# qdrant/qdrant

Hardware: AMD Instinct MI355X
Metric: QPS @ recall@10, brute-force, d=768 10M vecs, f32 cosine top-10 (higher is better)
Workload: dtype f32 (int8 prefilter + exact f32 re-score)

## Files before the change

### qdrant_amd/csrc/api_core.hip

```cpp
#include "api_internal.hpp"

namespace qmx {

static thread_local std::string g_last_error;
const std::string &last_error_text() { return g_last_error; }

void set_error(const char *fmt, ...) {
    char buf[1024];
    va_list ap;
    va_start(ap, fmt);
    vsnprintf(buf, sizeof(buf), fmt, ap);
    va_end(ap);
    g_last_error = buf;
}

int32_t hip_status(hipError_t e, const char *what, const char *file, int line) {
    set_error("HIP error %d (%s) at %s:%d: %s", (int)e, hipGetErrorString(e), file, line, what);
    (void)hipGetLastError();
    switch (e) {
        case hipErrorOutOfMemory: return QMX_ERR_OUT_OF_MEMORY;
        case hipErrorNoDevice:
        case hipErrorInvalidDevice:
        case hipErrorNoBinaryForGpu:
        case hipErrorInsufficientDriver: return QMX_ERR_NO_DEVICE;
        case hipErrorNotReady: return QMX_ERR_NOT_READY;
        case hipErrorInvalidValue: return QMX_ERR_BAD_ARG;
        default: return QMX_ERR_OTHER;
    }
}

static const char *const g_option_names[OPT_COUNT] = {"no_mfma_scan", "no_mfma16", "no_prescan", "prescan_shift", "hnsw_log_cap", "no_split_scan", "split_min_queries", "no_split256", "no_pq_pair", "no_pq_prefilter", "pq_prefilter_min_queries", "hnsw_pq_per_cu", "tq_rotate_block", "no_topk_small", "verify_max_per_query", "hnsw_pq_direct_walk", "hnsw_pq_table_build", "hnsw_no_pq_prefilter", "hnsw_no_lds_visited", "pq_lut_no_lds", "hnsw_per_cu", "hnsw_reference_heap_order", "tq_wide_min_queries", "tq_wide_high_digit", "sq_wide_min_queries", "i8_resident", "debug"};
struct OptionTable {
    std::atomic<int64_t> v[OPT_COUNT];
    int64_t initial[OPT_COUNT];
    OptionTable() {
        for (int i = 0; i < OPT_COUNT; ++i) {
            char env[64] = "QMX_";
            size_t k = 4;
            for (const char *c = g_option_names[i]; *c && k + 1 < sizeof(env); ++c) env[k++] = (char)toupper((unsigned char)*c);
            env[k] = 0;
            const char *e = getenv(env);
            int64_t val = 0;
            if (e) { val = (*e >= '0' && *e <= '9') ? atoll(e) : 1; }
            if (i == OPT_PRESCAN_SHIFT && !e) val = 10;
            if (i == OPT_SPLIT_MIN_QUERIES && !e) val = 1;
            if (i == OPT_PQ_PREFILTER_MIN_QUERIES && !e) val = 4;
            if (i == OPT_TQ_WIDE_MIN_QUERIES && !e) val = 33;
            if (i == OPT_SQ_WIDE_MIN_QUERIES && !e) val = 33;
            if (i == OPT_I8_RESIDENT && !e) val = 1;
            initial[i] = val;
            v[i].store(val, std::memory_order_relaxed);
        }
    }
};
static OptionTable g_options;
int64_t option(Option o) { return g_options.v[o].load(std::memory_order_relaxed); }

static thread_local const void *g_last_kernel = nullptr;
const void *last_noted_kernel() { return g_last_kernel; }
void note_kernel(const void *host_function) { g_last_kernel = host_function; }

void clear_stale_error() {
    hipError_t e = hipGetLastError();
    if (e != hipSuccess) {
        const bool debug = option(OPT_DEBUG) != 0;
        if (debug) fprintf(stderr, "[qmx] dropped stale HIP error %d (%s) before a kernel launch\n", (int)e, hipGetErrorString(e));
    }
}

bool is_device_ptr(const void *p) {
    if (!p) return false;
    hipPointerAttribute_t attr;
// ... 90 lines not shown
```

### qdrant_amd/csrc/api_internal.hpp

```cpp
#pragma once
#include <stdarg.h>
#include <stdio.h>
#include <stdlib.h>
#include <string.h>

#include <ctype.h>
#include <cxxabi.h>

#include <algorithm>
#include <atomic>
#include <mutex>
#include <string>
#include <thread>
#include <new>
#include <vector>

#include "kernels.hpp"
#include "tq_rotate.hpp"

namespace qmx {
const std::string &last_error_text();
const void *last_noted_kernel();
bool is_device_ptr(const void *p);
uint32_t elem_bytes(uint32_t dtype);
// ... 345 lines not shown
    DeletedView del;
};

struct CustomWalk {
    const qmx_custom_query *d_desc;
    const float *d_coefs;
    uint32_t n_queries, max_examples;
    uint32_t lds_bytes = 0;
};

static bool tq_l1(const qmx_segment *s) { return s->dtype == QMX_DTYPE_TQ && s->distance == QMX_DISTANCE_MANHATTAN; }

extern "C" {
int32_t hnsw_enqueue(const qmx_hnsw *g, qmx_query *q, uint32_t top, uint32_t ef, qmx_scored_point *d_out,
                            uint32_t *d_counts, uint32_t *d_scored, bool timed, bool acorn = false, const MultiWalk *mw = nullptr,
                            const ExpandedOut *xo = nullptr, const CustomWalk *cw = nullptr, const PopTrace *pt = nullptr);
int32_t hnsw_check(const qmx_hnsw *g, const qmx_query *q, uint32_t top, uint32_t ef);
int32_t hnsw_search_sync(const qmx_hnsw *g, qmx_query *q, uint32_t top, uint32_t ef, qmx_scored_point *out, uint32_t *out_counts,
                                const volatile uint8_t *is_stopped, qmx_counters *counters, bool acorn);
void fill_args(const qmx_query *q, uint32_t tile0, uint32_t nq_tile, ScanArgs &a);
int32_t launch_scan(const qmx_query *q, int qt, ScanMode mode, const ScanArgs &a, uint32_t *grid);
int32_t tq_l1_scores_device(qmx_query *q, uint32_t q0, uint32_t nq, const uint32_t *d_ids, uint64_t n, float *d_scores, uint64_t stride, const PairSel *sel);
int32_t score_matrix_enqueue(const qmx_query *q, uint32_t tile0, uint32_t nq_tile, const uint32_t *d_ids, uint64_t n, float *d_scores, uint64_t stride,
                                    uint32_t *launches);
int32_t score_ids_device(qmx_query *q, const uint32_t *d_ids, uint64_t n, float *d_scores, qmx_counters *counters);
int32_t score_pairs_device(qmx_query *q, const PairSel &sel, const uint32_t *d_ids, uint64_t n_items, float *d_scores,
                                  bool timed);
int32_t search_enqueue(qmx_query *q, uint32_t top, const uint32_t *d_ids, uint64_t n_ids,
                              qmx_scored_point *d_out, uint32_t *d_counts, const volatile uint8_t *is_stopped,
                              qmx_counters *counters, bool timed);
int32_t fold_split_counters(qmx_query *q, qmx_counters *c);
int32_t custom_validate(const qmx_query *ex, const qmx_custom_query *queries, uint32_t n_queries, uint32_t n_examples, uint32_t *max_examples);
TqRotationHost tq_rotation(const qmx_segment *s);
TqRotationHost tq_rotation_inverse(const qmx_segment *s);
}
void sparse_segment_free(qmx_segment *s);
void sparse_query_free(qmx_query *q);
int32_t sparse_query_create_internal(const qmx_segment *seg, const uint32_t *point_ids, uint32_t nq, qmx_query **out);
int32_t sparse_score_matrix(const qmx_query *q, uint32_t tile0, uint32_t nq_tile, const uint32_t *d_ids, uint64_t n, float *d_scores, uint64_t stride);
int32_t sparse_score_pairs(qmx_query *q, const PairSel &sel, const uint32_t *d_ids, uint64_t n_items, float *d_scores);
int32_t sparse_score_internal(const qmx_segment *seg, const uint32_t *a_ids, const uint32_t *b_ids, uint32_t n, float *out);
int32_t sparse_search_enqueue(qmx_query *q, uint32_t top, const uint32_t *d_ids, uint64_t n_ids, qmx_scored_point *d_out, uint32_t *d_counts,
                              const volatile uint8_t *is_stopped, qmx_counters *counters, bool timed);
```

### qdrant_amd/csrc/api_query.hip

```cpp
#include "api_internal.hpp"

extern "C" {

static int32_t query_alloc(const qmx_segment *seg, uint32_t nq, qmx_query **out, bool internal = false) {
    qmx_query *q = new (std::nothrow) qmx_query();
    QMX_REQUIRE(q, QMX_ERR_OUT_OF_MEMORY, "host allocation failed");
    q->seg = seg;
    q->device = seg->device;
    q->nq = nq;
    q->nq_padded = ((nq + MAX_QT_TOPK - 1) / MAX_QT_TOPK) * MAX_QT_TOPK;
    if (q->nq_padded == 0) q->nq_padded = MAX_QT_TOPK;
    if (seg->dtype == QMX_DTYPE_PQ) q->nq_padded = std::max<uint32_t>(nq, 1);
    q->bq_bits = (seg->dtype == QMX_DTYPE_BQ && !internal) ? seg->bq_query_bits : 1;
    q->aux_off = (uint32_t)((seg->scan_dim * elem_bytes(seg->dtype) * q->bq_bits + 127) & ~127u);
    if (seg->dtype == QMX_DTYPE_TQ) tq_entry_layout(seg, &q->bq_bits, &q->tq_qbytes_off, &q->aux_off);
    if (seg->dtype == QMX_DTYPE_BQ && q->bq_bits > 1 && seg->fast_layout()) {
        q->tq_qbytes_off = q->aux_off;
        q->aux_off += ((seg->scan_dim + 63) & ~63u) * 8;
    }
    q->q_stride = q->aux_off + QUERY_AUX_BYTES;
    if (seg->dtype == QMX_DTYPE_SQ_U8 || seg->dtype == QMX_DTYPE_F16 || seg->dtype == QMX_DTYPE_TQ || (seg->dtype == QMX_DTYPE_BQ && q->tq_qbytes_off))
        q->q_stride = lds_tile_stride(q->q_stride);
    if (seg->dtype == QMX_DTYPE_PQ) {
        q->q_stride = (uint32_t)(((size_t)seg->pq_m * seg->pq.n_centroids * sizeof(float) + 15) & ~(size_t)15);
// ... 335 lines not shown
    }
    set_error("dtype %u not built yet", s->dtype);
    return QMX_ERR_NOT_SUPPORTED;
}

int32_t tq_l1_scores_device(qmx_query *q, uint32_t q0, uint32_t nq, const uint32_t *d_ids, uint64_t n, float *d_scores, uint64_t stride, const PairSel *sel) {
    const qmx_segment *s = q->seg;
    const uint64_t B = 65536;
    QMX_TRY(q->tq_rot.reserve((size_t)std::min<uint64_t>(n, B) * s->tq_padded_dim * sizeof(double)));
    double *buf = (double *)q->tq_rot.p;
    const float *d_q = (const float *)q->enc.p + (size_t)q0 * s->dim;
    for (uint64_t r0 = 0; r0 < n; r0 += B) {
        const uint32_t cnt = (uint32_t)std::min<uint64_t>(B, n - r0);
        QMX_TRY(launch_tq_l1_dequant(q->stream, s->d_rows, s->row_stride, s->d_tq_sf, d_ids ? d_ids + r0 : nullptr, r0, cnt, s->n, s->tq_padded_dim, s->tq_value_bits,
                                     s->d_tq_shift, s->d_tq_scale, buf, q->d_err, sel));
        QMX_TRY(launch_tq_rotate_f64(q->stream, buf, cnt, tq_rotation_inverse(s)));
        QMX_TRY(launch_tq_l1_scores(q->stream, buf, cnt, s->tq_padded_dim, s->dim, sel ? (const float *)q->enc.p : d_q, s->dim, 0, nq, d_scores, stride, r0,
                                    s->tq_invert ? 1 : 0, sel, r0));
    }
    return QMX_OK;
}

int32_t score_matrix_enqueue(const qmx_query *q, uint32_t tile0, uint32_t nq_tile, const uint32_t *d_ids, uint64_t n, float *d_scores, uint64_t stride,
                                    uint32_t *launches) {
    const qmx_segment *s = q->seg;
    if (is_sparse(s)) {
        if (launches) ++*launches;
        return sparse_score_matrix(q, tile0, nq_tile, d_ids, n, d_scores, stride);
    }
    if (tq_l1(s)) {
        if (launches) *launches += 3 * (uint32_t)((n + 65535) / 65536);
        return tq_l1_scores_device(const_cast<qmx_query *>(q), tile0, nq_tile, d_ids, n, d_scores, stride, nullptr);
    }
    const uint32_t SQT = tile_qt(s, q);
    const bool loops = s->dtype == QMX_DTYPE_F32 && SQT >= 8 && mfma_scan_ok(s);
    const uint32_t step = loops ? nq_tile : SQT;
    for (uint32_t st0 = 0; st0 < nq_tile; st0 += step) {
        const uint32_t nq_sub = std::min<uint32_t>(step, nq_tile - st0);
        ScanArgs pre;
        fill_args(q, tile0 + st0, nq_sub, pre);
        pre.ids = d_ids;
        pre.n_cand = n;
        pre.top = 1;
        pre.scores = d_scores + (size_t)st0 * stride;
        pre.scores_stride = stride;
        uint32_t pgrid = 0;
        QMX_TRY(launch_scan(q, (int)std::min<uint32_t>(pow2_ceil(nq_sub), std::max<uint32_t>(SQT, 8)), SCAN_SCORES, pre, &pgrid));
        if (launches) ++*launches;
    }
    return QMX_OK;
}

int32_t score_ids_device(qmx_query *q, const uint32_t *d_ids, uint64_t n, float *d_scores, qmx_counters *counters) {
    const qmx_segment *s = q->seg;
    const uint32_t TQ = tile_qt(s, q);
    uint32_t launches = 0;
    QMX_TRY(score_matrix_enqueue(q, 0, q->nq, d_ids, n, d_scores, n, &launches));
    if (counters) {
        counters->kernel_launches += launches;
        counters->vectors_scored += (uint64_t)q->nq * n;
        counters->bytes_read += (uint64_t)((q->nq + TQ - 1) / TQ) * n * s->row_bytes;
    }
    return QMX_OK;
}

int32_t qmx_score_points(qmx_query *q, const uint32_t *ids, uint32_t n, float *scores, qmx_counters *counters) {
    QMX_REQUIRE(q && (n == 0 || (ids && scores)), QMX_ERR_BAD_ARG, "NULL argument");
    QMX_HIP(hipSetDevice(q->seg->device));
    if (counters) memset(counters, 0, sizeof(*counters));
    if (n == 0 || q->nq == 0) return QMX_OK;
// ... 269 lines not shown
```

### qdrant_amd/csrc/api_search.hip

```cpp
#include "api_internal.hpp"

extern "C" {



static int32_t split_stage(qmx_query *q, const char *what) {
    if (option(OPT_DEBUG) < 2) return QMX_OK;
    hipError_t e = hipStreamSynchronize(q->stream);
    fprintf(stderr, "[qmx] split stage %-28s %s\n", what, e == hipSuccess ? "ok" : hipGetErrorString(e));
    fflush(stderr);
    return e == hipSuccess ? QMX_OK : QMX_ERR_OTHER;
}

static int32_t verify_pool(qmx_query *q, unsigned char *plan, VerifyPool *vp) {
    const uint32_t cap = (uint32_t)std::min<uint64_t>(std::max<uint64_t>((uint64_t)q->nq * SPLIT_VCAP, 262144), 1u << 26);
    QMX_TRY(q->sp_ver.reserve(((size_t)cap * 2 + (size_t)q->nq * 2) * 4));
    QMX_TRY(q->sp_vscores.reserve((size_t)cap * 4));
    uint32_t *b = (uint32_t *)q->sp_ver.p;
    vp->ids = b;
    vp->qsel = b + cap;
    vp->off = b + (size_t)2 * cap;
    vp->cnt = vp->off + q->nq;
    vp->used = (uint32_t *)(plan + 24);
    vp->cap = cap;
// ... 344 lines not shown
            ::qmx::clear_stale_error();
            hipLaunchKernelGGL(sample_ids_kernel, dim3((uint32_t)((S + 255) / 256)), dim3(256), 0, q->stream, (uint32_t *)q->sp_sample.p, (uint32_t)S, n_cand / S);
            QMX_HIP(hipGetLastError());
            q->sp_sample_n = S;
            q->sp_sample_of = n_cand;
        }
        QMX_HIP(hipMemsetAsync(plan, 0, pl.zero_bytes, q->stream));
    }
    for (uint32_t tile0 = 0; tile0 < q->nq; tile0 += TQ) {
        const uint32_t nq_tile = std::min<uint32_t>(TQ, q->nq - tile0);
        if (split && (nq_tile > MAX_QT_TOPK || s->d_rows_split)) {
            if (is_stopped && *is_stopped) {
                set_error("search cancelled");
                return QMX_ERR_CANCELLED;
            }
            const uint32_t S = (uint32_t)q->sp_sample_n;
            const uint32_t *d_sample = (const uint32_t *)q->sp_sample.p;
            uint64_t *gthr = (uint64_t *)q->gthr.p + tile0;
            ScanArgs a;
            fill_args(q, tile0, nq_tile, a);
            a.n_cand = n_cand;
            a.top = top;
            QMX_TRY(q->scores.reserve((size_t)nq_tile * S * sizeof(float)));
            QMX_TRY(score_matrix_enqueue(q, tile0, nq_tile, d_sample, S, (float *)q->scores.p, S, nullptr));
            QMX_TRY(launch_custom_topk(q->stream, (const float *)q->scores.p, S, d_sample, a.del, nq_tile, top, d_out + (size_t)tile0 * top, d_counts + tile0, gthr));
            QMX_TRY(split_stage(q, "prescan"));
            if (s->split_i8) {
                float *sp_texact = sp_qnorm, *sp_qscale = sp_qmax;
                QMX_TRY(launch_split_i8_pack(q->stream, (const float *)q->enc.p + (size_t)tile0 * s->dim, nq_tile, s->dim, s->d_i8_scale, gthr, s->d_i8_stats,
                                             s->row_norm_max, q->sp_bq.p, sp_qscale, sp_band, sp_thr, sp_texact, (uint32_t *)q->sp_cnt.p, SPLIT_QT_MAX));
                QMX_TRY(split_stage(q, "int8 pack"));
                const uint32_t np = split_i8_probe();
                uint32_t *probe_ids = (uint32_t *)q->sp_probe.p, *probe_cnt = probe_ids + (size_t)q->nq * np;
                int *tile_ovf = (int *)(plan + pl.tile_ovf) + split_tiles.size();
                const uint32_t sstride = 16;
                for (uint32_t ph = 1; ph <= 2; ++ph) {
                    const uint32_t phase = ph | (sstride << 8);
                    size_t slot = 0;
                    if (timed) QMX_TRY(timing_begin(q, &slot));
                    QMX_TRY(launch_scan_i8copy(q->stream, a, q->sp_bq.p, sp_qscale, sp_thr, s->num_cus, s->d_rows_split, q->sp_wl.p, phase));
                    q->last_kernel = last_noted_kernel();
                    if (timed) QMX_TRY(timing_end(q, slot));
                    QMX_TRY(launch_split_regroup(q->stream, a, q->sp_wl.p, s->num_cus, (uint64_t *)q->sp_cand.p, (uint32_t *)q->sp_cnt.p, SPLIT_CAND_CAP, tile_ovf,
                                                 phase, SPLIT_QT));
                    QMX_TRY(launch_split_i8_probe(q->stream, (const uint64_t *)q->sp_cand.p, (const uint32_t *)q->sp_cnt.p, SPLIT_CAND_CAP, sp_band, nq_tile, top, tile_ovf,
                                                  probe_ids + (size_t)tile0 * np, probe_cnt + tile0));
                    const void *scan_kernel = q->last_kernel;
                    PairSel psel{nullptr, np, probe_cnt};
// ... 373 lines not shown
```

### qdrant_amd/csrc/common.hpp

```cpp
#pragma once
#include <hip/hip_runtime.h>
#include <hip/hip_fp16.h>
#include <stdint.h>
#include <atomic>
#include <string>

#include "../../include/qdrant_amd.h"

namespace qmx {

void set_error(const char *fmt, ...);
int32_t hip_status(hipError_t e, const char *what, const char *file, int line);
void clear_stale_error();

enum Option {
    OPT_NO_MFMA_SCAN = 0,
    OPT_NO_MFMA16,
    OPT_NO_PRESCAN,
    OPT_PRESCAN_SHIFT,
    OPT_HNSW_LOG_CAP,
    OPT_NO_SPLIT_SCAN,
    OPT_SPLIT_MIN_QUERIES,
    OPT_NO_SPLIT256,
    OPT_NO_PQ_PAIR,
    OPT_NO_PQ_PREFILTER,
    OPT_PQ_PREFILTER_MIN_QUERIES,
    OPT_HNSW_PQ_PER_CU,
    OPT_TQ_ROTATE_BLOCK,
    OPT_NO_TOPK_SMALL,
    OPT_VERIFY_MAX_PER_QUERY,
    OPT_HNSW_PQ_DIRECT_WALK,
    OPT_HNSW_PQ_TABLE_BUILD,
    OPT_HNSW_NO_PQ_PREFILTER,
    OPT_HNSW_NO_LDS_VISITED,
    OPT_PQ_LUT_NO_LDS,
    OPT_HNSW_PER_CU,
    OPT_HNSW_REFERENCE_HEAP_ORDER,
    OPT_TQ_WIDE_MIN_QUERIES,
    OPT_TQ_WIDE_HIGH_DIGIT,
    OPT_SQ_WIDE_MIN_QUERIES,
    OPT_I8_RESIDENT,
    OPT_DEBUG,
    OPT_COUNT
};
int64_t option(Option o);
struct DeviceOnce {
    std::atomic<uint64_t> done{0};
    int dev = 0;
    bool need() {
        if (hipGetDevice(&dev) != hipSuccess) { dev = 0; return true; }
        return dev >= 64 || !(done.load(std::memory_order_acquire) & (1ull << dev));
    }
    void mark() { if (dev < 64) done.fetch_or(1ull << dev, std::memory_order_release); }
};
void note_kernel(const void *host_function);
#define QMX_NOTE_KERNEL(fn) ::qmx::note_kernel(reinterpret_cast<const void *>(fn))

#define QMX_HIP(expr)                                                        \
    do {                                                                     \
        hipError_t e__ = (expr);                                             \
        if (e__ != hipSuccess) return ::qmx::hip_status(e__, #expr, __FILE__, __LINE__); \
    } while (0)

#define QMX_TRY(expr)                           \
// ... 99 lines not shown
```

### qdrant_amd/csrc/custom_query.hip

```cpp
#include "custom_combine.hpp"
#include "kernels.hpp"

namespace qmx {

__device__ __forceinline__ float custom_combine(const qmx_custom_query &q, const float *sims, uint64_t stride, const float *coefs) {
    const float *s = sims + (uint64_t)q.first * stride;
    return custom_score_by(q.kind, q.n_a, q.n_b, coefs + q.coef_first, [&](uint32_t e) { return s[(uint64_t)e * stride]; });
}

__global__ __launch_bounds__(256) void custom_combine_kernel(const qmx_custom_query *queries, uint32_t n_queries, const float *sims, uint64_t n,
                                                             const float *coefs, float *out) {
    const uint64_t c = (uint64_t)blockIdx.x * 256 + threadIdx.x;
    const uint32_t qi = blockIdx.y;
    if (c >= n || qi >= n_queries) return;
    out[(uint64_t)qi * n + c] = custom_combine(queries[qi], sims + c, n, coefs);
}

int32_t launch_custom_combine(hipStream_t st, const qmx_custom_query *d_queries, uint32_t n_queries, const float *d_sims, uint64_t n,
                              const float *d_coefs, float *d_out) {
    if (n == 0 || n_queries == 0) return QMX_OK;
    ::qmx::clear_stale_error();
    hipLaunchKernelGGL(custom_combine_kernel, dim3((uint32_t)((n + 255) / 256), n_queries), dim3(256), 0, st, d_queries, n_queries, d_sims, n, d_coefs, d_out);
    QMX_HIP(hipGetLastError());
    return QMX_OK;
// ... 124 lines not shown
            }
            const uint32_t cnt = (uint32_t)__popcll(__ballot(ok));
            if (lane == 0) {
                sh_bound = cnt == (uint32_t)ptop ? readlane_u64(merged, ptop - 1) : 0ull;
                total += cnt;
            }
            total = (uint32_t)__builtin_amdgcn_readfirstlane((int)total);
        }
        __syncthreads();
        bound = sh_bound;
        if (bound == 0) {
            for (uint32_t i = off + WAVE + threadIdx.x; i < top; i += CT_BLOCK) out[(uint64_t)q * top + i] = qmx_scored_point{0u, 0.0f};
            break;
        }
    }
    if (threadIdx.x == 0) {
        out_counts[q] = total;
        if (bound_out) bound_out[q] = total == top ? bound : 0ull;
    }
}

constexpr int CTS_E = 16;
constexpr uint64_t CTS_MAX_N = (uint64_t)CT_BLOCK * CTS_E;
__global__ __launch_bounds__(CT_BLOCK) void custom_topk_small_kernel(const float *scores, uint32_t n, const uint32_t *ids, DeletedView del, uint32_t top,
                                                                     qmx_scored_point *out, uint32_t *out_counts, uint64_t *bound_out) {
    extern __shared__ __attribute__((aligned(16))) unsigned char smem_cts[];
    uint64_t *surv = reinterpret_cast<uint64_t *>(smem_cts);
    __shared__ uint64_t sh_t[CT_NW];
    __shared__ uint64_t sh_bound;
    __shared__ uint32_t sh_cnt;
    const uint32_t q = blockIdx.x;
    const int lane = threadIdx.x & 63, wave = threadIdx.x >> 6;
    const float *row = scores + (uint64_t)q * n;
    uint64_t kreg[CTS_E];
#pragma unroll
    for (int e0 = 0; e0 < CTS_E; e0 += 8) {
        if ((uint32_t)e0 * CT_BLOCK >= n) {
#pragma unroll
            for (int u = 0; u < 8; ++u) kreg[e0 + u] = 0ull;
            continue;
        }
        uint32_t id[8];
        uint64_t key[8], keep[8];
#pragma unroll
        for (int u = 0; u < 8; ++u) {
            const uint32_t c = (uint32_t)(e0 + u) * CT_BLOCK + threadIdx.x;
            const uint32_t cc = c < n ? c : 0;
            id[u] = ids ? ids[cc] : cc;
            key[u] = c < n ? make_key(row[cc], id[u]) : 0ull;
        }
        live_masks<8>(del, id, keep);
#pragma unroll
        for (int u = 0; u < 8; ++u) kreg[e0 + u] = key[u] & keep[u];
    }
    uint64_t bound = ~0ull;
    uint32_t total = 0;
    for (uint32_t off = 0; off < top; off += WAVE) {
        const uint32_t ptop = top - off < (uint32_t)WAVE ? top - off : (uint32_t)WAVE;
        uint64_t m = 0;
#pragma unroll
        for (int e = 0; e < CTS_E; ++e) {
            const uint64_t k = kreg[e] < bound ? kreg[e] : 0ull;
            m = k > m ? k : m;
        }
        uint32_t rank = 0;
        for (int j = 0; j < WAVE; ++j) rank += readlane_u64(m, j) > m ? 1u : 0u;
        const uint64_t sel = __ballot(rank == ptop - 1 && m != 0);
        const uint64_t tw = sel ? readlane_u64(m, __builtin_ctzll(sel)) : 0ull;
        if (lane == 0) sh_t[wave] = tw;
        if (threadIdx.x == 0) { sh_cnt = 0; sh_bound = 0; }
        __syncthreads();
        uint64_t t = 0;
#pragma unroll
        for (int w = 0; w < CT_NW; ++w) t = sh_t[w] > t ? sh_t[w] : t;
#pragma unroll
        for (int e = 0; e < CTS_E; ++e) {
            const uint64_t k = kreg[e] < bound ? kreg[e] : 0ull;
            if (k != 0 && k >= t) surv[atomicAdd(&sh_cnt, 1u)] = k;
        }
        __syncthreads();
        const uint32_t cnt = sh_cnt;
        for (uint32_t i = threadIdx.x; i < cnt; i += CT_BLOCK) {
            const uint64_t my = surv[i];
            uint32_t r = 0;
            for (uint32_t j = 0; j < cnt; ++j) r += (surv[j] > my || (surv[j] == my && j < i)) ? 1u : 0u;
            if (r < ptop) {
                qmx_scored_point p;
                p.idx = key_idx(my);
                p.score = key_score(my);
                out[(uint64_t)q * top + off + r] = p;
                if (r == ptop - 1) sh_bound = my;
            }
        }
        const uint32_t found = cnt < ptop ? cnt : ptop;
        for (uint32_t i = found + threadIdx.x; i < ptop; i += CT_BLOCK) out[(uint64_t)q * top + off + i] = qmx_scored_point{0u, 0.0f};
        total += found;
        __syncthreads();
        bound = sh_bound;
        if (bound == 0) {
            for (uint32_t i = off + WAVE + threadIdx.x; i < top; i += CT_BLOCK) out[(uint64_t)q * top + i] = qmx_scored_point{0u, 0.0f};
            break;
        }
        __syncthreads();
    }
    if (threadIdx.x == 0) {
        out_counts[q] = total;
        if (bound_out) bound_out[q] = total == top ? bound : 0ull;
    }
}

int32_t launch_custom_topk(hipStream_t st, const float *d_scores, uint64_t n, const uint32_t *d_ids, const DeletedView &del, uint32_t n_queries,
                           uint32_t top, qmx_scored_point *d_out, uint32_t *d_counts, uint64_t *d_bound) {
    if (n_queries == 0) return QMX_OK;
    ::qmx::clear_stale_error();
    if (n >= 1 && n <= CTS_MAX_N && !option(OPT_NO_TOPK_SMALL)) {
        static thread_local DeviceOnce attr_once;
        if (attr_once.need()) {
            QMX_HIP(hipFuncSetAttribute(reinterpret_cast<const void *>(custom_topk_small_kernel), hipFuncAttributeMaxDynamicSharedMemorySize, (int)(CTS_MAX_N * 8)));
            attr_once.mark();
        }
        hipLaunchKernelGGL(custom_topk_small_kernel, dim3(n_queries), dim3(CT_BLOCK), (size_t)n * 8, st, d_scores, (uint32_t)n, d_ids, del, top, d_out, d_counts, d_bound);
        QMX_HIP(hipGetLastError());
        return QMX_OK;
    }
    hipLaunchKernelGGL(custom_topk_kernel, dim3(n_queries), dim3(CT_BLOCK), 0, st, d_scores, n, d_ids, del, top, d_out, d_counts, d_bound);
    QMX_HIP(hipGetLastError());
    return QMX_OK;
}

}
```

### qdrant_amd/csrc/kernels.hpp

```cpp
#pragma once
#include "common.hpp"

namespace qmx {

constexpr int MAX_QT = 16;
constexpr int SCAN_BLOCK = 512;
constexpr int MAX_TOP_FAST = 64;

struct TqEc {
    const int16_t *weights;
    const float *xm;
    float weight_scale, mm_const;
};
struct ScanArgs {
    const void *rows;
    uint64_t n_rows;
    uint64_t row_stride;
    uint32_t dim;
    uint32_t nseg;
    uint32_t rem_pieces;
    uint32_t tail_start;
    uint32_t aux_off;
    uint32_t nq;
    const void *queries;
// ... 196 lines not shown
    uint32_t *next;
};
int32_t launch_hnsw_build_bq(hipStream_t st, const ScanArgs &a, const HnswBuildArgs &h, int phase, uint32_t grid, int *per_cu);
int32_t launch_hnsw_build_sq(hipStream_t st, int distance, const ScanArgs &a, const HnswBuildArgs &h, int phase, uint32_t grid, int *per_cu);
int32_t launch_hnsw_build_dense(hipStream_t st, int dtype, int distance, const ScanArgs &a, const HnswBuildArgs &h, int phase,
                                uint32_t grid, int *per_cu);
int32_t launch_hnsw_build_maxsim_dense(hipStream_t st, int dtype, int distance, const ScanArgs &a, const HnswBuildArgs &h, int phase, uint32_t grid,
                                       int *per_cu);
int32_t launch_hnsw_build_maxsim_sq(hipStream_t st, int distance, const ScanArgs &a, const HnswBuildArgs &h, int phase, uint32_t grid, int *per_cu);
int32_t launch_hnsw_build_maxsim_bq(hipStream_t st, const ScanArgs &a, const HnswBuildArgs &h, int phase, uint32_t grid, int *per_cu);
int32_t launch_hnsw_build_tq(hipStream_t st, const ScanArgs &a, const HnswBuildArgs &h, int phase, uint32_t grid, int *per_cu);
int32_t launch_hnsw_build_tq_l1(hipStream_t st, const ScanArgs &a, const HnswBuildArgs &h, int phase, uint32_t grid, int *per_cu, uint32_t rot_dim,
                                uint32_t padded_dim);
int32_t launch_hnsw_build_pq(hipStream_t st, const ScanArgs &a, const HnswBuildArgs &h, int phase, uint32_t grid, int *per_cu);
int32_t launch_hnsw_build_maxsim_pq(hipStream_t st, const ScanArgs &a, const HnswBuildArgs &h, int phase, uint32_t grid, int *per_cu);
int32_t launch_hnsw_build_maxsim_tq(hipStream_t st, const ScanArgs &a, const HnswBuildArgs &h, int phase, uint32_t grid, int *per_cu);
int32_t launch_pq_pair_table(hipStream_t st, uint32_t distance, uint32_t dim, const qmx_pq_params &pq, const float *d_centroids, float *d_pair);
int32_t launch_u8_row_norms(hipStream_t st, const void *rows, uint64_t row_stride, uint64_t n, uint32_t dim, uint32_t flags, float *norms_f, int32_t *norms_i);
constexpr uint32_t HNSW_LDS_QUERY_MAX = 150 * 1024;

int32_t launch_scan_dense(hipStream_t st, int dtype, int distance, int qt, ScanMode mode,
                          const ScanArgs &a, int num_cus, uint32_t *grid_out);
int32_t launch_scan_f32_mfma(hipStream_t st, int qt, ScanMode mode, const ScanArgs &a, int num_cus, uint32_t *grid_out);
bool sq_mfma_ok(uint32_t distance, uint32_t actual_dim);
int32_t launch_scan_sq_mfma(hipStream_t st, int qt, ScanMode mode, const ScanArgs &a, int num_cus, uint32_t *grid_out);
int32_t launch_scan_f16_mfma(hipStream_t st, int qt, ScanMode mode, const ScanArgs &a, int num_cus, uint32_t *grid_out);
struct PairSel {
    const uint32_t *qsel;
    uint32_t per_query;
    const uint32_t *counts;
    const uint32_t *limit;
    __device__ __forceinline__ uint32_t query_of(uint64_t item) const {
        if (qsel) return qsel[item];
        if (per_query) return (uint32_t)(item / per_query);
        return (uint32_t)item;
    }
    __device__ __forceinline__ bool live(uint64_t item, uint32_t qi) const {
        if (limit && item >= (uint64_t)*limit) return false;
        if (per_query && counts) return (uint32_t)(item % per_query) < counts[qi];
        return true;
    }
};

int32_t launch_pairs_dense(hipStream_t st, int dtype, int distance, const ScanArgs &a, const PairSel &sel,
                           uint64_t n_items, int num_cus);
int32_t launch_pairs_sq(hipStream_t st, int distance, const ScanArgs &a, const PairSel &sel, uint64_t n_items, int num_cus);
// ... 47 lines not shown
    uint32_t fallback_queries;
    uint32_t pad;
};
struct VerifyPool {
    uint32_t *ids, *qsel, *off, *cnt, *used;
    uint32_t cap;
    uint32_t max_per_query;
};
int32_t launch_split_select(hipStream_t st, const uint64_t *d_cand, const uint32_t *d_cand_cnt, uint32_t cap, const float *d_band, uint32_t nq, uint32_t top,
                            const VerifyPool &pool, uint32_t q_base, const int *d_tile_overflow, uint32_t *d_ovf_q, SplitStats *d_stats,
                            const float *d_t_exact = nullptr, bool tighten = false);
bool split_i8_dim_ok(uint32_t dim);
size_t split_i8_copy_bytes(uint64_t n, uint32_t dim);
size_t split_i8_query_bytes(uint32_t dim);
uint32_t split_i8_probe();
int32_t launch_split_i8_colstats(hipStream_t st, const void *rows, uint64_t row_stride, uint64_t n, uint32_t dim, uint32_t *d_colmax, float *d_colsq);
float split_i8_choose_scales(const float *colmax, const float *colsq, uint64_t n, uint32_t dim, float *scale);
int32_t launch_split_i8_rowstats(hipStream_t st, const void *rows, uint64_t row_stride, uint64_t n, uint32_t dim, const float *d_scale, uint32_t *d_stats);
int32_t launch_split_i8_copy(hipStream_t st, const void *rows, uint64_t row_stride, uint64_t n, uint32_t dim, const float *d_scale, void *d_out);
int32_t launch_split_i8_pack(hipStream_t st, const float *d_q, uint32_t nq, uint32_t dim, const float *d_scale, const uint64_t *d_gthr, const uint32_t *d_row_stats,
                             float row_norm_max, void *d_bq, float *d_qscale, float *d_band, float *d_thr, float *d_t_exact, uint32_t *d_cand_cnt, uint32_t n_cnt);
int32_t launch_scan_i8copy(hipStream_t st, const ScanArgs &a, const void *d_bq, const float *d_qscale, const float *d_thr, int num_cus, const void *d_rows_i8,
                           void *d_wlists, uint32_t phase);
int32_t launch_split_i8_probe(hipStream_t st, const uint64_t *d_cand, const uint32_t *d_cand_cnt, uint32_t cap, const float *d_band, uint32_t nq, uint32_t top,
                              const int *d_tile_overflow, uint32_t *d_probe_ids, uint32_t *d_probe_cnt);
int32_t launch_split_i8_bound(hipStream_t st, const float *d_scores, uint32_t *d_probe_cnt, uint32_t nq, uint32_t top, const float *d_band, const float *d_qscale,
                              float *d_thr, float *d_t_exact);
bool tq4w_shape_ok(const ScanArgs &a);
size_t tq4w_query_bytes(uint32_t code_bytes);
size_t tq4w_wlists_counts_bytes(int num_cus);
size_t tq4w_wlists_bytes(int num_cus);
uint32_t tq4w_wcap();
int32_t launch_tq4w_stats(hipStream_t st, const float *d_sf, const float *d_l2, const void *d_rows, uint64_t row_stride, uint32_t code_bytes, uint64_t n, uint32_t *d_stats);
int32_t launch_tq4w_pack(hipStream_t st, const ScanArgs &a, const uint64_t *d_gthr, float sf_min, float sf_max, float l2_min, float l2_max, uint32_t c1, int high_only,
                         void *d_bq, int32_t *d_thr_i,
                         float *d_qinfo, float *d_band, uint32_t *d_cand_cnt, uint32_t n_cnt);
int32_t launch_scan_tq4w(hipStream_t st, const ScanArgs &a, const void *d_bq, const int32_t *d_thr_i, const float *d_qinfo, const float *d_band_high_only, int num_cus,
                         void *d_wlists, uint32_t *grid_out);
bool sqw_shape_ok(const ScanArgs &a);
size_t sqw_query_bytes(uint32_t dim);
size_t sqw_wlists_counts_bytes(int num_cus);
size_t sqw_wlists_bytes(int num_cus);
uint32_t sqw_wcap();
int32_t launch_sqw_stats(hipStream_t st, const float *d_off, uint64_t n, float multiplier, int32_t *d_bi, uint32_t *d_stats);
int32_t launch_sqw_pack(hipStream_t st, const ScanArgs &a, const uint64_t *d_gthr, float off_absmax, void *d_bq, int32_t *d_thr_i, float *d_qinfo, float *d_band,
                        uint32_t *d_cand_cnt, uint32_t n_cnt);
// ... 23 lines not shown
int32_t launch_pq_train(hipStream_t st, uint32_t dim, uint32_t chunk_size, uint32_t n_centroids, const float *d_data, uint64_t n,
                        uint32_t max_iters, float accuracy, uint32_t threads, float *d_centroids, uint32_t *iters_host);
int32_t launch_pq_encode(hipStream_t st, uint32_t dim, const qmx_pq_params &pq, const float *d_centroids, const float *d_in,
                         uint64_t n, uint8_t *d_codes);
int32_t launch_pack_queries(hipStream_t st, int dtype, int distance, const void *src, int src_is_encoded,
                            uint32_t src_stride, uint32_t nq, uint32_t dim, void *tile, uint32_t q_stride, uint32_t aux_off);
int32_t launch_merge_keys(hipStream_t st, const uint64_t *partial, uint32_t n_lists,
                          uint32_t qt_stride, uint32_t nq, uint32_t top, qmx_scored_point *out,
                          uint32_t *out_counts, uint32_t out_stride = 0, uint32_t out_offset = 0,
                          uint64_t *next_bound = nullptr, const int *run_if = nullptr, const uint32_t *out_map = nullptr, uint32_t shared_grid = 0);
int32_t launch_merge_points(hipStream_t st, const qmx_scored_point *lists, const uint32_t *list_counts,
                            const uint32_t *list_idx_base, uint32_t n_lists, uint32_t nq, uint32_t k, qmx_scored_point *out,
                            uint32_t *out_counts, uint64_t list_stride = 0, uint64_t count_stride = 0);
int32_t launch_split_candidates(hipStream_t st, const qmx_scored_point *cand, const uint32_t *cand_cnt, uint32_t n_per, uint32_t nq,
                                uint32_t *ids, uint32_t top, qmx_scored_point *out, uint32_t *out_counts);
int32_t launch_sort_scored(hipStream_t st, const float *scores, const uint32_t *ids, const uint32_t *counts, uint32_t n_per_query, uint32_t nq, uint32_t top,
                           qmx_scored_point *out, uint32_t *out_counts, const uint32_t *offsets = nullptr);

int32_t launch_custom_combine(hipStream_t st, const qmx_custom_query *d_queries, uint32_t n_queries, const float *d_sims, uint64_t n,
                              const float *d_coefs, float *d_out);
int32_t launch_maxsim(hipStream_t st, const float *d_sims, uint64_t n_rows, const uint32_t *d_qfirst, uint32_t n_queries, const uint64_t *d_offsets,
                      uint32_t n_points, const uint32_t *d_ids, uint64_t n, float *d_out, int *err_flag);
int32_t launch_custom_topk(hipStream_t st, const float *d_scores, uint64_t n, const uint32_t *d_ids, const DeletedView &del, uint32_t n_queries,
                           uint32_t top, qmx_scored_point *d_out, uint32_t *d_counts, uint64_t *d_bound = nullptr);

int32_t launch_cosine_preprocess_f32(hipStream_t st, const float *in, float *out, uint64_t n, uint32_t dim);
int32_t launch_cast_f32(hipStream_t st, int dst_dtype, const float *in, void *out, uint64_t count);
int32_t launch_minmax_f32(hipStream_t st, const float *in, uint64_t count, float *min_out, float *max_out);
int32_t launch_gather_rows(hipStream_t st, const void *rows, uint64_t row_stride, uint64_t row_bytes,
                           const uint32_t *ids, uint32_t n, uint64_t n_rows, void *out, int *err_flag);

struct SparseRows {
    const uint64_t *off;
    const uint32_t *idx;
    const float *val;
    uint64_t n;
};
struct SparseQueries {
    const uint64_t *off;
    const uint32_t *idx;
    const float *val;
};
struct SparsePlan {
    const uint32_t *off;
    const uint64_t *start;
    const uint64_t *end;
    const float *w;
// ... 59 lines not shown
```

### qdrant_amd/csrc/scan_mfma.hip

```cpp
#include "scan_common.hpp"

namespace qmx {

typedef float f32x4 __attribute__((ext_vector_type(4)));


template <int XORMASK>
__device__ __forceinline__ float swz_xor(float v) {
    return __int_as_float(__builtin_amdgcn_ds_swizzle(__float_as_int(v), (XORMASK << 10) | 0x1F));
}
__device__ __forceinline__ float ror8(float v) {
    return __int_as_float(__builtin_amdgcn_update_dpp(0, __float_as_int(v), 0x128 , 0xF, 0xF, true));
}
__device__ __forceinline__ float swap16_add(float a, float b) {
    const auto r = __builtin_amdgcn_permlane16_swap(__float_as_uint(a), __float_as_uint(b), false, false);
    return __uint_as_float(r[0]) + __uint_as_float(r[1]);
}

template <int QW, int QSPLIT, int D, bool NT, int NWAVES, bool FAST, bool QH, bool HAS_IDS, int MODE>
__device__ __forceinline__ void scan_f32_mfma_body(const ScanArgs &a, unsigned char *smem) {
    constexpr int MF_BLOCK = NWAVES * 64, MF_NW = NWAVES;
    constexpr int GQ = QH ? 8 : 4;
    constexpr int TR = QH ? 4 : 8;
    constexpr int NG = QW / GQ;
// ... 320 lines not shown
    switch (qt) {
        case 8: return launch_mfma_qt<8, 1, 4, true>(st, mode, a, num_cus, grid_out);
        case 16:
            if (mfma16_scan_ok(16, mode, a)) return launch_scan_f32_mfma16(st, 16, a, num_cus, grid_out);
            if (a.nseg % 12 == 0) return launch_mfma_qt<16, 1, 6, true, 8, true>(st, mode, a, num_cus, grid_out);
            return launch_mfma_qt<16, 1, 12, true>(st, mode, a, num_cus, grid_out);
        case 32: {
            if (mfma16_scan_ok(32, mode, a)) return launch_scan_f32_mfma16(st, 32, a, num_cus, grid_out);
#ifdef QMX_TUNING
            static const int variant = getenv("QMX_MFMA_VARIANT") ? atoi(getenv("QMX_MFMA_VARIANT")) : 0;
            if (variant == 1) return launch_mfma_qt<32, 1, 6, true, 8, false, true>(st, mode, a, num_cus, grid_out);
            if (variant == 2 && a.nseg % 12 == 0) return launch_mfma_qt<32, 1, 6, true, 8, true, true>(st, mode, a, num_cus, grid_out);
            if (variant == 3 && a.nseg % 24 == 0) return launch_mfma_qt<32, 1, 12, true, 8, true, true>(st, mode, a, num_cus, grid_out);
#endif
            if (a.nseg % 12 == 0) return launch_mfma_qt<16, 2, 6, true, 8, true>(st, mode, a, num_cus, grid_out);
            return launch_mfma_qt<16, 2, 12, true>(st, mode, a, num_cus, grid_out);
        }
    }
    if (qt == 64 && mfma16_scan_ok(64, mode, a)) return launch_scan_f32_mfma16(st, 64, a, num_cus, grid_out);
    set_error("unsupported MFMA query tile %d", qt);
    return QMX_ERR_BAD_ARG;
}

}
```

### qdrant_amd/csrc/scan_split.hip

```cpp
#include <type_traits>

#include "scan_common.hpp"

namespace qmx {

typedef _Float16 half8 __attribute__((ext_vector_type(8)));
typedef _Float16 half4 __attribute__((ext_vector_type(4)));
typedef float f32x4s __attribute__((ext_vector_type(4)));

constexpr int SP_BM = 256;
constexpr int SP_QT = 128;
constexpr int SP_QT_MAX = 256;
constexpr int SP_THREADS = 768;
constexpr int SP_CONSUMERS = 8;
constexpr int SP_A_UNITS = SP_BM * 2 * 4;
constexpr int SP_B_UNITS = SP_QT * 2 * 4;
constexpr int SP_BRING = 4;
constexpr int SP_LDS = (2 * SP_A_UNITS + SP_BRING * SP_B_UNITS) * 16;

__device__ __forceinline__ uint32_t sp_unit(uint32_t t, uint32_t hl, uint32_t kq, uint32_t m) { return ((t * 2 + hl) * 4 + kq) * 16 + (m ^ (2 * kq)); }

__device__ __forceinline__ void sp_split4(const f32x4s v, float scale, half4 &h, half4 &l) {
#pragma unroll
    for (int i = 0; i < 4; ++i) {
// ... 1735 lines not shown
    QMX_REQUIRE(split_i8_dim_ok(dim), QMX_ERR_BAD_ARG, "int8 copy of dim %u", dim);
    ::qmx::clear_stale_error();
    QMX_HIP(hipMemsetAsync(d_stats, 0, 16, st));
    if (n) hipLaunchKernelGGL(sp_i8_row_stats_kernel, dim3(2048), dim3(256), 0, st, (const unsigned char *)rows, row_stride, n, dim, d_scale, d_stats);
    QMX_HIP(hipGetLastError());
    return QMX_OK;
}
int32_t launch_split_i8_copy(hipStream_t st, const void *rows, uint64_t row_stride, uint64_t n, uint32_t dim, const float *d_scale, void *d_out) {
    if (n == 0) return QMX_OK;
    ::qmx::clear_stale_error();
    hipLaunchKernelGGL(sp_i8_copy_kernel, dim3(8192), dim3(256), 0, st, (const unsigned char *)rows, row_stride, n, dim, d_scale, (uint4 *)d_out);
    QMX_HIP(hipGetLastError());
    return QMX_OK;
}
int32_t launch_split_i8_pack(hipStream_t st, const float *d_q, uint32_t nq, uint32_t dim, const float *d_scale, const uint64_t *d_gthr, const uint32_t *d_row_stats,
                             float row_norm_max, void *d_bq, float *d_qscale, float *d_band, float *d_thr, float *d_t_exact, uint32_t *d_cand_cnt, uint32_t n_cnt) {
    QMX_REQUIRE(nq <= (uint32_t)SP_QT, QMX_ERR_BAD_ARG, "int8 tile of %u queries", nq);
    ::qmx::clear_stale_error();
    hipLaunchKernelGGL(sp_i8_pack_kernel, dim3(SP_QT), dim3(256), (size_t)dim * 4, st, d_q, nq, dim, d_scale, d_gthr, d_row_stats, row_norm_max, (uint4 *)d_bq,
                       d_qscale, d_band, d_thr, d_t_exact, d_cand_cnt, n_cnt);
    QMX_HIP(hipGetLastError());
    return QMX_OK;
}
int32_t launch_scan_i8copy(hipStream_t st, const ScanArgs &a, const void *d_bq, const float *d_qscale, const float *d_thr, int num_cus, const void *d_rows_i8,
                           void *d_wlists, uint32_t phase) {
    const uint32_t nch_r = a.dim / 128;
    const bool resident = option(OPT_I8_RESIDENT) > 0 && nch_r <= SP8R_MAX_NCH;
    void (*kfn)(const ScanArgs, const SplitArgs) = resident ? scan_i8copy_kernel_res<1> : scan_i8copy_kernel;
    const size_t lds_bytes = resident ? sp8r_lds_bytes(nch_r) : (size_t)SP8_LDS;
    static thread_local DeviceOnce attr_once;
    if (attr_once.need()) {
        QMX_HIP(hipFuncSetAttribute(reinterpret_cast<const void *>(scan_i8copy_kernel), hipFuncAttributeMaxDynamicSharedMemorySize, SP8_LDS));
        QMX_HIP(hipFuncSetAttribute(reinterpret_cast<const void *>(scan_i8copy_kernel_res<1>), hipFuncAttributeMaxDynamicSharedMemorySize, (int)sp8r_lds_bytes(SP8R_MAX_NCH)));
        attr_once.mark();
    }
    QMX_REQUIRE(d_rows_i8 && d_wlists && split_i8_dim_ok(a.dim), QMX_ERR_BAD_ARG, "the int8 scan reads the int8 copy and writes per-wave candidate lists");
    SplitArgs s;
    s.rows_split = (const uint4 *)d_rows_i8;
    s.bq = (const uint4 *)d_bq;
    s.nchunks = a.dim / 128;
    s.nq = a.nq;
    s.row_scale = 1.0f;
    s.scales = d_qscale;
    s.thr = d_thr;
    s.cand = nullptr;
    s.cand_cnt = nullptr;
    s.cap = 0;
    s.wcap = SP_WCAP;
    s.wcnt = (uint32_t *)d_wlists;
    s.wlist = (uint4 *)((unsigned char *)d_wlists + split_wlists_counts_bytes(num_cus));
// ... 27 lines not shown
```

Before: 98290.

## Run sample prescan and top-k with small-LDS variants to co-reside with int8 scan

Adds a default-on option that, in the split int8 path, scores the sample with a lighter f32 MFMA scan configuration (16-query tile, small LDS footprint). It also runs the sample top-k with a 256-thread, 32-element-per-thread variant whose survivor buffer is capped to a small LDS size. The aim is to let these prescan kernels fit in LDS alongside the resident int8 scan kernel, so they can overlap or co-schedule on the same CUs instead of serialising. The trade-off is a less efficient MFMA tile for the sample scan and a capped survivor list in top-k that may truncate candidates if more ties survive than the cap.

```diff
diff --git a/qdrant_amd/csrc/api_core.hip b/qdrant_amd/csrc/api_core.hip
--- a/qdrant_amd/csrc/api_core.hip
+++ b/qdrant_amd/csrc/api_core.hip
@@ -29,7 +29,7 @@
     }
 }
 
-static const char *const g_option_names[OPT_COUNT] = {"no_mfma_scan", "no_mfma16", "no_prescan", "prescan_shift", "hnsw_log_cap", "no_split_scan", "split_min_queries", "no_split256", "no_pq_pair", "no_pq_prefilter", "pq_prefilter_min_queries", "hnsw_pq_per_cu", "tq_rotate_block", "no_topk_small", "verify_max_per_query", "hnsw_pq_direct_walk", "hnsw_pq_table_build", "hnsw_no_pq_prefilter", "hnsw_no_lds_visited", "pq_lut_no_lds", "hnsw_per_cu", "hnsw_reference_heap_order", "tq_wide_min_queries", "tq_wide_high_digit", "sq_wide_min_queries", "i8_resident", "debug"};
+static const char *const g_option_names[OPT_COUNT] = {"no_mfma_scan", "no_mfma16", "no_prescan", "prescan_shift", "hnsw_log_cap", "no_split_scan", "split_min_queries", "no_split256", "no_pq_pair", "no_pq_prefilter", "pq_prefilter_min_queries", "hnsw_pq_per_cu", "tq_rotate_block", "no_topk_small", "verify_max_per_query", "hnsw_pq_direct_walk", "hnsw_pq_table_build", "hnsw_no_pq_prefilter", "hnsw_no_lds_visited", "pq_lut_no_lds", "hnsw_per_cu", "hnsw_reference_heap_order", "tq_wide_min_queries", "tq_wide_high_digit", "sq_wide_min_queries", "i8_resident", "sample_beside_scan", "debug"};
 struct OptionTable {
     std::atomic<int64_t> v[OPT_COUNT];
     int64_t initial[OPT_COUNT];
@@ -48,6 +48,7 @@
             if (i == OPT_TQ_WIDE_MIN_QUERIES && !e) val = 33;
             if (i == OPT_SQ_WIDE_MIN_QUERIES && !e) val = 33;
             if (i == OPT_I8_RESIDENT && !e) val = 1;
+            if (i == OPT_SAMPLE_BESIDE_SCAN && !e) val = 1;
             initial[i] = val;
             v[i].store(val, std::memory_order_relaxed);
         }
diff --git a/qdrant_amd/csrc/api_internal.hpp b/qdrant_amd/csrc/api_internal.hpp
--- a/qdrant_amd/csrc/api_internal.hpp
+++ b/qdrant_amd/csrc/api_internal.hpp
@@ -391,7 +391,7 @@
 int32_t launch_scan(const qmx_query *q, int qt, ScanMode mode, const ScanArgs &a, uint32_t *grid);
 int32_t tq_l1_scores_device(qmx_query *q, uint32_t q0, uint32_t nq, const uint32_t *d_ids, uint64_t n, float *d_scores, uint64_t stride, const PairSel *sel);
 int32_t score_matrix_enqueue(const qmx_query *q, uint32_t tile0, uint32_t nq_tile, const uint32_t *d_ids, uint64_t n, float *d_scores, uint64_t stride,
-                                    uint32_t *launches);
+                                    uint32_t *launches, bool beside_scan = false);
 int32_t score_ids_device(qmx_query *q, const uint32_t *d_ids, uint64_t n, float *d_scores, qmx_counters *counters);
 int32_t score_pairs_device(qmx_query *q, const PairSel &sel, const uint32_t *d_ids, uint64_t n_items, float *d_scores,
                                   bool timed);
diff --git a/qdrant_amd/csrc/api_query.hip b/qdrant_amd/csrc/api_query.hip
--- a/qdrant_amd/csrc/api_query.hip
+++ b/qdrant_amd/csrc/api_query.hip
@@ -381,7 +381,7 @@
 }
 
 int32_t score_matrix_enqueue(const qmx_query *q, uint32_t tile0, uint32_t nq_tile, const uint32_t *d_ids, uint64_t n, float *d_scores, uint64_t stride,
-                                    uint32_t *launches) {
+                                    uint32_t *launches, bool beside_scan) {
     const qmx_segment *s = q->seg;
     if (is_sparse(s)) {
         if (launches) ++*launches;
@@ -394,6 +394,7 @@
     const uint32_t SQT = tile_qt(s, q);
     const bool loops = s->dtype == QMX_DTYPE_F32 && SQT >= 8 && mfma_scan_ok(s);
     const uint32_t step = loops ? nq_tile : SQT;
+    const bool beside = loops && nq_tile > 8 && (beside_scan || option(OPT_SAMPLE_BESIDE_SCAN) >= 2);
     for (uint32_t st0 = 0; st0 < nq_tile; st0 += step) {
         const uint32_t nq_sub = std::min<uint32_t>(step, nq_tile - st0);
         ScanArgs pre;
@@ -404,7 +405,10 @@
         pre.scores = d_scores + (size_t)st0 * stride;
         pre.scores_stride = stride;
         uint32_t pgrid = 0;
-        QMX_TRY(launch_scan(q, (int)std::min<uint32_t>(pow2_ceil(nq_sub), std::max<uint32_t>(SQT, 8)), SCAN_SCORES, pre, &pgrid));
+        if (beside)
+            QMX_TRY(launch_scan_f32_mfma_beside(q->stream, pre, s->num_cus));
+        else
+            QMX_TRY(launch_scan(q, (int)std::min<uint32_t>(pow2_ceil(nq_sub), std::max<uint32_t>(SQT, 8)), SCAN_SCORES, pre, &pgrid));
         if (launches) ++*launches;
     }
     return QMX_OK;
diff --git a/qdrant_amd/csrc/api_search.hip b/qdrant_amd/csrc/api_search.hip
--- a/qdrant_amd/csrc/api_search.hip
+++ b/qdrant_amd/csrc/api_search.hip
@@ -390,8 +390,11 @@
             a.n_cand = n_cand;
             a.top = top;
             QMX_TRY(q->scores.reserve((size_t)nq_tile * S * sizeof(float)));
-            QMX_TRY(score_matrix_enqueue(q, tile0, nq_tile, d_sample, S, (float *)q->scores.p, S, nullptr));
-            QMX_TRY(launch_custom_topk(q->stream, (const float *)q->scores.p, S, d_sample, a.del, nq_tile, top, d_out + (size_t)tile0 * top, d_counts + tile0, gthr));
+            const size_t scan_lds = s->split_i8 ? split_i8_resident_lds(s->dim) : 0;
+            const bool beside_scan = option(OPT_SAMPLE_BESIDE_SCAN) > 0 && scan_lds != 0 && scan_f32_mfma_beside_lds(a) + scan_lds + 4096 <= 160 * 1024;
+            QMX_TRY(score_matrix_enqueue(q, tile0, nq_tile, d_sample, S, (float *)q->scores.p, S, nullptr, beside_scan));
+            QMX_TRY(launch_custom_topk(q->stream, (const float *)q->scores.p, S, d_sample, a.del, nq_tile, top, d_out + (size_t)tile0 * top, d_counts + tile0, gthr,
+                                       beside_scan));
             QMX_TRY(split_stage(q, "prescan"));
             if (s->split_i8) {
                 float *sp_texact = sp_qnorm, *sp_qscale = sp_qmax;
diff --git a/qdrant_amd/csrc/common.hpp b/qdrant_amd/csrc/common.hpp
--- a/qdrant_amd/csrc/common.hpp
+++ b/qdrant_amd/csrc/common.hpp
@@ -40,6 +40,7 @@
     OPT_TQ_WIDE_HIGH_DIGIT,
     OPT_SQ_WIDE_MIN_QUERIES,
     OPT_I8_RESIDENT,
+    OPT_SAMPLE_BESIDE_SCAN,
     OPT_DEBUG,
     OPT_COUNT
 };
diff --git a/qdrant_amd/csrc/custom_query.hip b/qdrant_amd/csrc/custom_query.hip
--- a/qdrant_amd/csrc/custom_query.hip
+++ b/qdrant_amd/csrc/custom_query.hip
@@ -170,20 +170,23 @@
 
 constexpr int CTS_E = 16;
 constexpr uint64_t CTS_MAX_N = (uint64_t)CT_BLOCK * CTS_E;
-__global__ __launch_bounds__(CT_BLOCK) void custom_topk_small_kernel(const float *scores, uint32_t n, const uint32_t *ids, DeletedView del, uint32_t top,
-                                                                     qmx_scored_point *out, uint32_t *out_counts, uint64_t *bound_out) {
+constexpr int CTS_BESIDE_BLOCK = 256, CTS_BESIDE_E = 32;
+template <int BLOCK, int E>
+__global__ __launch_bounds__(BLOCK) void custom_topk_small_kernel(const float *scores, uint32_t n, const uint32_t *ids, DeletedView del, uint32_t top,
+                                                                  qmx_scored_point *out, uint32_t *out_counts, uint64_t *bound_out, uint32_t cap) {
+    constexpr int NW = BLOCK / WAVE;
     extern __shared__ __attribute__((aligned(16))) unsigned char smem_cts[];
     uint64_t *surv = reinterpret_cast<uint64_t *>(smem_cts);
-    __shared__ uint64_t sh_t[CT_NW];
+    __shared__ uint64_t sh_t[NW];
     __shared__ uint64_t sh_bound;
     __shared__ uint32_t sh_cnt;
     const uint32_t q = blockIdx.x;
     const int lane = threadIdx.x & 63, wave = threadIdx.x >> 6;
     const float *row = scores + (uint64_t)q * n;
-    uint64_t kreg[CTS_E];
-#pragma unroll
-    for (int e0 = 0; e0 < CTS_E; e0 += 8) {
-        if ((uint32_t)e0 * CT_BLOCK >= n) {
+    uint64_t kreg[E];
+#pragma unroll
+    for (int e0 = 0; e0 < E; e0 += 8) {
+        if ((uint32_t)e0 * BLOCK >= n) {
 #pragma unroll
             for (int u = 0; u < 8; ++u) kreg[e0 + u] = 0ull;
             continue;
@@ -192,7 +195,7 @@
         uint64_t key[8], keep[8];
 #pragma unroll
         for (int u = 0; u < 8; ++u) {
-            const uint32_t c = (uint32_t)(e0 + u) * CT_BLOCK + threadIdx.x;
+            const uint32_t c = (uint32_t)(e0 + u) * BLOCK + threadIdx.x;
             const uint32_t cc = c < n ? c : 0;
             id[u] = ids ? ids[cc] : cc;
             key[u] = c < n ? make_key(row[cc], id[u]) : 0ull;
@@ -207,7 +210,7 @@
         const uint32_t ptop = top - off < (uint32_t)WAVE ? top - off : (uint32_t)WAVE;
         uint64_t m = 0;
 #pragma unroll
-        for (int e = 0; e < CTS_E; ++e) {
+        for (int e = 0; e < E; ++e) {
             const uint64_t k = kreg[e] < bound ? kreg[e] : 0ull;
             m = k > m ? k : m;
         }
@@ -220,15 +223,18 @@
         __syncthreads();
         uint64_t t = 0;
 #pragma unroll
-        for (int w = 0; w < CT_NW; ++w) t = sh_t[w] > t ? sh_t[w] : t;
-#pragma unroll
-        for (int e = 0; e < CTS_E; ++e) {
+        for (int w = 0; w < NW; ++w) t = sh_t[w] > t ? sh_t[w] : t;
+#pragma unroll
+        for (int e = 0; e < E; ++e) {
             const uint64_t k = kreg[e] < bound ? kreg[e] : 0ull;
-            if (k != 0 && k >= t) surv[atomicAdd(&sh_cnt, 1u)] = k;
-        }
-        __syncthreads();
-        const uint32_t cnt = sh_cnt;
-        for (uint32_t i = threadIdx.x; i < cnt; i += CT_BLOCK) {
+            if (k != 0 && k >= t) {
+                const uint32_t at = atomicAdd(&sh_cnt, 1u);
+                if (at < cap) surv[at] = k;
+            }
+        }
+        __syncthreads();
+        const uint32_t cnt = sh_cnt < cap ? sh_cnt : cap;
+        for (uint32_t i = threadIdx.x; i < cnt; i += BLOCK) {
             const uint64_t my = surv[i];
             uint32_t r = 0;
             for (uint32_t j = 0; j < cnt; ++j) r += (surv[j] > my || (surv[j] == my && j < i)) ? 1u : 0u;
@@ -241,12 +247,12 @@
             }
         }
         const uint32_t found = cnt < ptop ? cnt : ptop;
-        for (uint32_t i = found + threadIdx.x; i < ptop; i += CT_BLOCK) out[(uint64_t)q * top + off + i] = qmx_scored_point{0u, 0.0f};
+        for (uint32_t i = found + threadIdx.x; i < ptop; i += BLOCK) out[(uint64_t)q * top + off + i] = qmx_scored_point{0u, 0.0f};
         total += found;
         __syncthreads();
         bound = sh_bound;
         if (bound == 0) {
-            for (uint32_t i = off + WAVE + threadIdx.x; i < top; i += CT_BLOCK) out[(uint64_t)q * top + i] = qmx_scored_point{0u, 0.0f};
+            for (uint32_t i = off + WAVE + threadIdx.x; i < top; i += BLOCK) out[(uint64_t)q * top + i] = qmx_scored_point{0u, 0.0f};
             break;
         }
         __syncthreads();
@@ -258,16 +264,25 @@
 }
 
 int32_t launch_custom_topk(hipStream_t st, const float *d_scores, uint64_t n, const uint32_t *d_ids, const DeletedView &del, uint32_t n_queries,
-                           uint32_t top, qmx_scored_point *d_out, uint32_t *d_counts, uint64_t *d_bound) {
+                           uint32_t top, qmx_scored_point *d_out, uint32_t *d_counts, uint64_t *d_bound, bool beside_scan) {
     if (n_queries == 0) return QMX_OK;
     ::qmx::clear_stale_error();
+    const uint64_t per_pass = (uint64_t)(CTS_BESIDE_BLOCK / WAVE) * std::min<uint32_t>(std::max<uint32_t>(top, 1), WAVE) * CTS_BESIDE_E;
+    const uint32_t cap = (uint32_t)std::min<uint64_t>(n, per_pass);
+    if (beside_scan && n >= 1 && n <= (uint64_t)CTS_BESIDE_BLOCK * CTS_BESIDE_E && (size_t)cap * 8 <= 32 * 1024 && !option(OPT_NO_TOPK_SMALL)) {
+        hipLaunchKernelGGL((custom_topk_small_kernel<CTS_BESIDE_BLOCK, CTS_BESIDE_E>), dim3(n_queries), dim3(CTS_BESIDE_BLOCK), (size_t)cap * 8, st, d_scores, (uint32_t)n,
+                           d_ids, del, top, d_out, d_counts, d_bound, cap);
+        QMX_HIP(hipGetLastError());
+        return QMX_OK;
+    }
     if (n >= 1 && n <= CTS_MAX_N && !option(OPT_NO_TOPK_SMALL)) {
+        auto kfn = custom_topk_small_kernel<CT_BLOCK, CTS_E>;
         static thread_local DeviceOnce attr_once;
         if (attr_once.need()) {
-            QMX_HIP(hipFuncSetAttribute(reinterpret_cast<const void *>(custom_topk_small_kernel), hipFuncAttributeMaxDynamicSharedMemorySize, (int)(CTS_MAX_N * 8)));
+            QMX_HIP(hipFuncSetAttribute(reinterpret_cast<const void *>(kfn), hipFuncAttributeMaxDynamicSharedMemorySize, (int)(CTS_MAX_N * 8)));
             attr_once.mark();
         }
-        hipLaunchKernelGGL(custom_topk_small_kernel, dim3(n_queries), dim3(CT_BLOCK), (size_t)n * 8, st, d_scores, (uint32_t)n, d_ids, del, top, d_out, d_counts, d_bound);
+        hipLaunchKernelGGL(kfn, dim3(n_queries), dim3(CT_BLOCK), (size_t)n * 8, st, d_scores, (uint32_t)n, d_ids, del, top, d_out, d_counts, d_bound, (uint32_t)n);
         QMX_HIP(hipGetLastError());
         return QMX_OK;
     }
diff --git a/qdrant_amd/csrc/kernels.hpp b/qdrant_amd/csrc/kernels.hpp
--- a/qdrant_amd/csrc/kernels.hpp
+++ b/qdrant_amd/csrc/kernels.hpp
@@ -242,6 +242,8 @@
 int32_t launch_scan_dense(hipStream_t st, int dtype, int distance, int qt, ScanMode mode,
                           const ScanArgs &a, int num_cus, uint32_t *grid_out);
 int32_t launch_scan_f32_mfma(hipStream_t st, int qt, ScanMode mode, const ScanArgs &a, int num_cus, uint32_t *grid_out);
+size_t scan_f32_mfma_beside_lds(const ScanArgs &a);
+int32_t launch_scan_f32_mfma_beside(hipStream_t st, const ScanArgs &a, int num_cus);
 bool sq_mfma_ok(uint32_t distance, uint32_t actual_dim);
 int32_t launch_scan_sq_mfma(hipStream_t st, int qt, ScanMode mode, const ScanArgs &a, int num_cus, uint32_t *grid_out);
 int32_t launch_scan_f16_mfma(hipStream_t st, int qt, ScanMode mode, const ScanArgs &a, int num_cus, uint32_t *grid_out);
@@ -335,6 +337,7 @@
                              float row_norm_max, void *d_bq, float *d_qscale, float *d_band, float *d_thr, float *d_t_exact, uint32_t *d_cand_cnt, uint32_t n_cnt);
 int32_t launch_scan_i8copy(hipStream_t st, const ScanArgs &a, const void *d_bq, const float *d_qscale, const float *d_thr, int num_cus, const void *d_rows_i8,
                            void *d_wlists, uint32_t phase);
+size_t split_i8_resident_lds(uint32_t dim);
 int32_t launch_split_i8_probe(hipStream_t st, const uint64_t *d_cand, const uint32_t *d_cand_cnt, uint32_t cap, const float *d_band, uint32_t nq, uint32_t top,
                               const int *d_tile_overflow, uint32_t *d_probe_ids, uint32_t *d_probe_cnt);
 int32_t launch_split_i8_bound(hipStream_t st, const float *d_scores, uint32_t *d_probe_cnt, uint32_t nq, uint32_t top, const float *d_band, const float *d_qscale,
@@ -404,7 +407,8 @@
 int32_t launch_maxsim(hipStream_t st, const float *d_sims, uint64_t n_rows, const uint32_t *d_qfirst, uint32_t n_queries, const uint64_t *d_offsets,
                       uint32_t n_points, const uint32_t *d_ids, uint64_t n, float *d_out, int *err_flag);
 int32_t launch_custom_topk(hipStream_t st, const float *d_scores, uint64_t n, const uint32_t *d_ids, const DeletedView &del, uint32_t n_queries,
-                           uint32_t top, qmx_scored_point *d_out, uint32_t *d_counts, uint64_t *d_bound = nullptr);
+                           uint32_t top, qmx_scored_point *d_out, uint32_t *d_counts, uint64_t *d_bound = nullptr,
+                           bool beside_scan = false);
 
 int32_t launch_cosine_preprocess_f32(hipStream_t st, const float *in, float *out, uint64_t n, uint32_t dim);
 int32_t launch_cast_f32(hipStream_t st, int dst_dtype, const float *in, void *out, uint64_t count);
diff --git a/qdrant_amd/csrc/scan_mfma.hip b/qdrant_amd/csrc/scan_mfma.hip
--- a/qdrant_amd/csrc/scan_mfma.hip
+++ b/qdrant_amd/csrc/scan_mfma.hip
@@ -366,4 +366,15 @@
     return QMX_ERR_BAD_ARG;
 }
 
-}
+size_t scan_f32_mfma_beside_lds(const ScanArgs &a) { return ((size_t)16 * a.q_stride + 256 + 15) & ~(size_t)15; }
+int32_t launch_scan_f32_mfma_beside(hipStream_t st, const ScanArgs &a, int num_cus) {
+    uint32_t grid = 0;
+    const bool ids = a.ids != nullptr;
+    if (a.nseg % 12 == 0)
+        return ids ? launch_mfma_inst<16, 1, 6, true, 4, true, false, true, SCAN_SCORES>(st, a, num_cus, &grid)
+                   : launch_mfma_inst<16, 1, 6, true, 4, true, false, false, SCAN_SCORES>(st, a, num_cus, &grid);
+    return ids ? launch_mfma_inst<16, 1, 4, true, 4, false, false, true, SCAN_SCORES>(st, a, num_cus, &grid)
+               : launch_mfma_inst<16, 1, 4, true, 4, false, false, false, SCAN_SCORES>(st, a, num_cus, &grid);
+}
+
+}
diff --git a/qdrant_amd/csrc/scan_split.hip b/qdrant_amd/csrc/scan_split.hip
--- a/qdrant_amd/csrc/scan_split.hip
+++ b/qdrant_amd/csrc/scan_split.hip
@@ -1781,10 +1781,11 @@
     QMX_HIP(hipGetLastError());
     return QMX_OK;
 }
+size_t split_i8_resident_lds(uint32_t dim) { return option(OPT_I8_RESIDENT) > 0 && dim / 128 <= SP8R_MAX_NCH ? sp8r_lds_bytes(dim / 128) : 0; }
 int32_t launch_scan_i8copy(hipStream_t st, const ScanArgs &a, const void *d_bq, const float *d_qscale, const float *d_thr, int num_cus, const void *d_rows_i8,
                            void *d_wlists, uint32_t phase) {
     const uint32_t nch_r = a.dim / 128;
-    const bool resident = option(OPT_I8_RESIDENT) > 0 && nch_r <= SP8R_MAX_NCH;
+    const bool resident = split_i8_resident_lds(a.dim) != 0;
     void (*kfn)(const ScanArgs, const SplitArgs) = resident ? scan_i8copy_kernel_res<1> : scan_i8copy_kernel;
     const size_t lds_bytes = resident ? sp8r_lds_bytes(nch_r) : (size_t)SP8_LDS;
     static thread_local DeviceOnce attr_once;
```

Result: no change. 98480, median of 6 (+0.2%).
